# mnastorg/PSI-GNN

Hardware: AMD Instinct MI355X
Metric: fixed-point edges/sec (E' x Broyden iterations/sec) on 1M-node Poisson mesh (higher is better)
Workload: dtype f32

## Files before the change

### psi-gnn_amd/csrc/common.h

```cpp
#pragma once
#include <hip/hip_runtime.h>
#include <stdint.h>
#include <stdio.h>
#include <string>
#include "../../include/psignn_hip.h"

#define D PSIGNN_D

void psignn_set_error(const char* fmt, ...);

extern int g_knob_epoch;
#define KNOB_INT(var, expr)                   \
  static int var##_epoch = -1;                \
  static int var = 0;                         \
  if (var##_epoch != g_knob_epoch) {          \
    var = (expr);                             \
    var##_epoch = g_knob_epoch;               \
  }

#define HIP_TRY(expr)                                                                   \
  do {                                                                                  \
    hipError_t _e = (expr);                                                             \
    if (_e != hipSuccess) {                                                             \
      psignn_set_error("%s:%d: %s -> %s", __FILE__, __LINE__, #expr, hipGetErrorString(_e)); \
// ... 111 lines not shown
    __VA_ARGS__;                         \
    if (g_prof_on) prof_end(st);         \
  } while (0)

#define FLAG_DIRICHLET 1
#define FLAG_NEUMANN 2

struct BatchDesc {
  int64_t M, ld;
  int32_t nblk, npart, nblk_ax, jgroups, thr, seq_len, keep_trace, n_tiles, tile_base;
  int32_t* st;
  float *U, *V, *xbuf, *g0, *g1, *upd, *part, *coef, *nrm_part, *jpart;
  double *rel_trace, *abs_trace;
  const struct TileCtx* ctx;
  const float *h0p, *prbp;
  float* part2;
  int32_t nblk_u, npart_u;
  float* parta;
  int32_t nblk4, pad_;
  const float* nrmp;
  int64_t pstride;
};

static inline size_t tile_lds_min() {
  KNOB_INT(mn, [] { const char* e = getenv("PSIGNN_TILE_LDS_MIN"); return e ? atoi(e) : 0; }());
  return (size_t)(mn < 0 ? 0 : (mn > 65536 ? 65536 : mn));
}
```

### psi-gnn_amd/csrc/fgnn_tile.hip

```cpp
#ifndef MV2_LAUNDER
#define MV2_LAUNDER 2
#endif
#ifndef MV2_CH
#define MV2_CH 10
#endif
#include "tile_helpers.h"
#ifndef TILE_WPE
#define TILE_WPE 0
#endif
#ifndef FUSED_WPE
#define FUSED_WPE 0
#endif
#if FUSED_WPE
#define TILE_WPE_ATTR __attribute__((amdgpu_waves_per_eu(FUSED ? FUSED_WPE : 1, FUSED ? FUSED_WPE : 8)))
#elif TILE_WPE
#define TILE_WPE_ATTR __attribute__((amdgpu_waves_per_eu(TILE_WPE, TILE_WPE)))
#else
#define TILE_WPE_ATTR
#endif
#ifndef X_RELOAD
#define X_RELOAD 1
#endif
#ifndef EDGE_CLAMP
#define EDGE_CLAMP 1
#endif
#ifndef EDGE_BOTH
#define EDGE_BOTH 1
#endif

// ... 38 lines not shown
#include <string.h>
#include <algorithm>
static int stage1_mfma(bool fused, bool mixed) {
  KNOB_INT(forced, [] {
    const char* e = getenv("PSIGNN_STAGE1");
    return !e ? -1 : (strcmp(e, "mfma") == 0 ? 1 : 0);
  }());
  if (forced >= 0) return forced;
  (void)fused;
  (void)mixed;
  return 0;
}

struct FuseArgs {
  const float* upd;
  float* gnew;
  float* xbuf;
  const int32_t* st;
  int off_done, off_cur, off_nxt;
  int64_t M;
  float* part;
  int npart;
  long long* stamps;
};

#ifndef TILE_PRIO
#define TILE_PRIO 15
#endif
#define PRIO_AT(ph) do { if (TILE_PRIO) __builtin_amdgcn_s_setprio((TILE_PRIO >> (2 * (ph))) & 3); } while (0)
#ifndef TILE_STAMPS
#define TILE_STAMPS 0
#endif
#if !TILE_STAMPS
#define STAMP(i) do { } while (0)
#else
#define STAMP(i)                                                                                        \
  do {                                                                                                  \
    if (fa.stamps && (threadIdx.x & 63) == 0)                                                           \
      fa.stamps[((int64_t)tile * 4 + (threadIdx.x >> 6)) * 8 + (i)] = (long long)wall_clock64(); \
  } while (0)
#endif
static long long* g_tile_stamps = nullptr;
extern "C" void psignn_prof_tile_stamps(void* d_buf) { g_tile_stamps = (long long*)d_buf; }

template <int CTRL>
__device__ __forceinline__ float dpp_perm_f(float v) {
// ... 473 lines not shown
  }
}

#ifndef TILE_CTX_VALUE
#define TILE_CTX_VALUE 1
#endif
#if TILE_CTX_VALUE
#define TILE_CTX_PARAM const TileCtx Cv
#define TILE_CTX_USE const TileCtx* __restrict__ C = &Cv;
#else
#define TILE_CTX_PARAM const TileCtx* __restrict__ C
#define TILE_CTX_USE
#endif
template <int P, bool MIXED, bool FUSED, bool MFMA1>
__global__ __launch_bounds__(TILE_THREADS) TILE_WPE_ATTR void k_f_tile(FuseArgs fa, int n_tiles, int chunk, const int32_t* __restrict__ tile_list,
                                                TILE_CTX_PARAM, const float* __restrict__ W, int lofs, int tofs,
                                                int tnofs, int apply_ln, const float* __restrict__ h,
                                                const int32_t* __restrict__ hsel, int64_t hstride,
                                                const float* __restrict__ h0, const float* __restrict__ prb,
                                                const float* __restrict__ nrm, float* __restrict__ out) {
  TILE_CTX_USE
  extern __shared__ __attribute__((aligned(16))) float lds[];
  if (FUSED && fa.st[fa.off_done]) return;
  const int slot = (blockIdx.x & 7) * chunk + (blockIdx.x >> 3);
  if (slot >= n_tiles) return;
  f_tile_body<P, MIXED, FUSED, MFMA1>(fa, slot, tile_list, C, W, lofs, tofs, tnofs, apply_ln, h, hsel, hstride, h0, prb, nrm, out,
                                      lds);
}

static unsigned tile_grid(int chunk);

#ifndef BATCH_WPE
#define BATCH_WPE 0
#endif
#if BATCH_WPE
#define BATCH_WPE_ATTR __attribute__((amdgpu_waves_per_eu(BATCH_WPE, BATCH_WPE)))
#else
#define BATCH_WPE_ATTR
#endif
template <int P, bool MIXED>
__global__ __launch_bounds__(TILE_THREADS) BATCH_WPE_ATTR void k_f_tile_batch(const BatchDesc* __restrict__ descs, int n_mesh, int n_slots, int chunk,
                                                              int off_done, int off_cur, int off_nxt, int par,
                                                              const float* __restrict__ W, int lofs, int tofs, int tnofs) {
  extern __shared__ __attribute__((aligned(16))) float lds[];
  const int slot = (blockIdx.x & 7) * chunk + (blockIdx.x >> 3);
  if (slot >= n_slots) return;
  int m = 0;
  while (m + 1 < n_mesh && descs[m + 1].tile_base <= slot) ++m;
  const BatchDesc& d = descs[m];
  if (d.st[off_done]) return;
  FuseArgs fa{d.upd, par ? d.g0 : d.g1, d.xbuf, d.st, off_done, off_cur, off_nxt, d.M, d.nrm_part, d.n_tiles, nullptr};
  f_tile_body<P, MIXED, true, false>(fa, slot - d.tile_base, nullptr, d.ctx, W, lofs, tofs, tnofs, 1, d.xbuf, nullptr, 0, d.h0p, d.prbp,
                                     d.nrmp, nullptr, lds);
}

int psignn_f_tile_fused_batch(const BatchDesc* d_descs, int n_mesh, int n_slots, int max_rows, const float* W, int mixed,
                              int off_done, int off_cur, int off_nxt, int par, hipStream_t st) {
  const int chunk = (int)cdiv(n_slots, 8);
  if (mixed) {
    using L = WLayout<3>;
    LAUNCH("k_f_tile_fused", st, (k_f_tile_batch<3, true><<<tile_grid(chunk), TILE_THREADS, (size_t)max_rows * TileRow<true>::RS * 4, st>>>(
        d_descs, n_mesh, n_slots, chunk, off_done, off_cur, off_nxt, par, W, L::layer(0), L::tp_layer(1, true, 0), L::tp_neu(1))));
  } else {
    using L = WLayout<2>;
    LAUNCH("k_f_tile_fused", st, (k_f_tile_batch<2, false><<<tile_grid(chunk), TILE_THREADS, (size_t)max_rows * TileRow<false>::RS * 4, st>>>(
        d_descs, n_mesh, n_slots, chunk, off_done, off_cur, off_nxt, par, W, L::layer(0), L::tp_layer(1, false, 0), 0)));
  }
  HIP_TRY(hipGetLastError());
  return PSIGNN_OK;
}

__global__ void k_permute_rows(int64_t N, int cols, const int32_t* __restrict__ map, const float* __restrict__ src,
                               float* __restrict__ dst) {
  int64_t i = (int64_t)blockIdx.x * blockDim.x + threadIdx.x;
// ... 21 lines not shown
      hipMemcpy(tsl.data(), p->tile_slice, (nt + 1) * 4, hipMemcpyDeviceToHost) != hipSuccess ||
      hipMemcpy(hc.data(), p->halo_cnt, nt * 4, hipMemcpyDeviceToHost) != hipSuccess ||
      hipMemcpy(deg.data(), p->slice_deg, p->n_slices, hipMemcpyDeviceToHost) != hipSuccess)
    return nullptr;
  std::vector<int64_t> cost(nt);
  for (int64_t t = 0; t < nt; ++t) {
    int dmax = 0;
    for (int s = tsl[t]; s < tsl[t + 1]; ++s) dmax = std::max(dmax, (int)deg[s]);
    cost[t] = (int64_t)(tptr[t + 1] - tptr[t] + hc[t]) + 16 * (int64_t)dmax;
  }
  for (int64_t t = 0; t < nt; ++t) order[t] = (int32_t)t;
  for (int x = 0; x < 8; ++x) {
    const int64_t a = std::min<int64_t>(nt, (int64_t)x * chunk), b = std::min<int64_t>(nt, (int64_t)(x + 1) * chunk);
    std::stable_sort(order.begin() + a, order.begin() + b, [&](int32_t u, int32_t v) { return cost[u] > cost[v]; });
  }
  int32_t* d = nullptr;
  if (hipMalloc((void**)&d, nt * 4) != hipSuccess) return nullptr;
  if (hipMemcpy(d, order.data(), nt * 4, hipMemcpyHostToDevice) != hipSuccess) { (void)hipFree(d); return nullptr; }
  p->tile_order_cost = d;
  (void)st;
  return d;
}

static FuseArgs plain_args() {
  FuseArgs a{};
  a.stamps = g_tile_stamps;
  return a;
}

template <bool FUSED>
static void launch_mixed(const psignn_plan* p, const FuseArgs& fa, const char* name, const float* W, int nl, const float* h,
                         const int32_t* hsel, int64_t hstride, const float* h0, const float* prb, const float* nrm,
                         float* out, hipStream_t st) {
  using L = WLayout<3>;
  const int lofs = L::layer(nl - 1), tofs = L::tp_layer(nl, true, nl - 1), tnofs = L::tp_neu(nl);
  int na = (int)p->n_tiles_plain, nb = (int)(p->n_tiles - p->n_tiles_plain);
  const char* e = getenv("PSIGNN_MIXED_SPLIT_MIN");
  if (na < (e ? atoi(e) : 2048)) {
    na = 0;
    nb = (int)p->n_tiles;
  }
  const int32_t* list_b = na > 0 ? p->tile_order + na : nullptr;
  if (na > 0) {
    const int chunk = (int)cdiv(na, 8);
    LAUNCH(name, st, (k_f_tile<3, false, FUSED, false><<<tile_grid(chunk), TILE_THREADS, (size_t)p->max_rows * TileRow<false>::RS * 4, st>>>(
        fa, na, chunk, p->tile_order, TILE_ARGS, W, lofs, tofs, tnofs, 1, h, hsel, hstride, h0, prb, nrm, out)));
  }
  if (nb > 0) {
    const int chunk = (int)cdiv(nb, 8);
    LAUNCH(name, st, (k_f_tile<3, true, FUSED, false><<<tile_grid(chunk), TILE_THREADS, (size_t)p->max_rows * TileRow<true>::RS * 4, st>>>(
        fa, nb, chunk, list_b, TILE_ARGS, W, lofs, tofs, tnofs, 1, h, hsel, hstride, h0, prb, nrm, out)));
  }
}

int psignn_f_tile_forward(const psignn_plan* p, const float* W, int nl, const float* h, const int32_t* hsel,
                          int64_t hstride, const float* h0, const float* prb, const float* nrm, float* out,
                          float* work, hipStream_t st) {
  ARG_CHECK(p && p->tiled, "plan has no tile structures");
  ARG_CHECK(W && h && h0 && prb && out, "NULL argument");
  ARG_CHECK(!p->mixed || nrm, "mixed plan needs unit normals");
  const int chunk = (int)cdiv(p->n_tiles, 8);
  const unsigned grid = tile_grid(chunk);
  PROF_BYTES(((p->mixed ? 102 : 89) * p->N + 20 * p->Ep) * (p->mixed ? 1 : nl));
  if (p->mixed) {
    using L = WLayout<3>;
    if (stage1_mfma(false, true)) {
      size_t lds = (size_t)p->max_rows * TileRow<true>::RS * 4;
      LAUNCH("k_f_tile", st, (k_f_tile<3, true, false, true><<<grid, TILE_THREADS, lds, st>>>(
        plain_args(), (int)p->n_tiles, chunk, nullptr, TILE_ARGS, W, L::layer(nl - 1), L::tp_layer(nl, true, nl - 1), L::tp_neu(nl), 1,
        h, hsel, hstride, h0, prb, nrm, out)));
    } else {
      launch_mixed<false>(p, plain_args(), "k_f_tile", W, nl, h, hsel, hstride, h0, prb, nrm, out, st);
    }
// ... 25 lines not shown
                        float* out, hipStream_t st) {
  ARG_CHECK(p && p->tiled && !p->mixed && l >= 0 && l < nl, "tiled layer: dirichlet plans, 0 <= layer < n_layers");
  ARG_CHECK(W && h && h0 && prb && out && out != h, "bad arguments");
  using L = WLayout<2>;
  const int chunk = (int)cdiv(p->n_tiles, 8);
  const unsigned grid = tile_grid(chunk);
  size_t lds = std::max((size_t)p->max_rows * TileRow<false>::RS * 4, tile_lds_min());
  const int32_t* tlist = tile_cost_order(p, chunk, st);
  PROF_BYTES(89 * p->N + 20 * p->Ep);
  if (stage1_mfma(false, false))
    LAUNCH("k_f_tile_layer", st, (k_f_tile<2, false, false, true><<<grid, TILE_THREADS, lds, st>>>(
        plain_args(), (int)p->n_tiles, chunk, tlist, TILE_ARGS, W, L::layer(l), L::tp_layer(nl, false, l), 0, l == nl - 1, h,
        nullptr, 0, h0, prb, nullptr, out)));
  else
    LAUNCH("k_f_tile_layer", st, (k_f_tile<2, false, false, false><<<grid, TILE_THREADS, lds, st>>>(
        plain_args(), (int)p->n_tiles, chunk, tlist, TILE_ARGS, W, L::layer(l), L::tp_layer(nl, false, l), 0, l == nl - 1, h,
        nullptr, 0, h0, prb, nullptr, out)));
  HIP_TRY(hipGetLastError());
  return PSIGNN_OK;
}

int psignn_f_tile_fused(const psignn_plan* p, const float* W, int nl, float* xbuf, int64_t M, const int32_t* st_words,
                        int off_done, int off_cur, int off_nxt, const float* upd, float* gnew,
                        const float* h0, const float* prb, const float* nrm, float* part, hipStream_t st) {
  ARG_CHECK(p && p->tiled, "plan has no tile structures");
  ARG_CHECK(nl == 1 || p->mixed, "fused step supports single-layer evaluation");
  const int chunk = (int)cdiv(p->n_tiles, 8);
  const unsigned grid = tile_grid(chunk);
  const int npart = (int)p->n_tiles;
  FuseArgs fa{upd, gnew, xbuf, st_words, off_done, off_cur, off_nxt, M, part, npart, g_tile_stamps};
  PROF_BYTES((p->mixed ? 102 : 89) * p->N + 20 * p->Ep + 8 * M);
  if (p->mixed) {
    using L = WLayout<3>;
    if (stage1_mfma(true, true)) {
      size_t lds = (size_t)p->max_rows * TileRow<true>::RS * 4;
      LAUNCH("k_f_tile_fused", st, (k_f_tile<3, true, true, true><<<grid, TILE_THREADS, lds, st>>>(
        fa, (int)p->n_tiles, chunk, nullptr, TILE_ARGS, W, L::layer(nl - 1), L::tp_layer(nl, true, nl - 1), L::tp_neu(nl), 1, xbuf,
        nullptr, 0, h0, prb, nrm, nullptr)));
    } else {
      launch_mixed<true>(p, fa, "k_f_tile_fused", W, nl, xbuf, nullptr, 0, h0, prb, nrm, nullptr, st);
    }
  } else {
    using L = WLayout<2>;
    size_t lds = std::max((size_t)p->max_rows * TileRow<false>::RS * 4, tile_lds_min());
    const int32_t* tlist = tile_cost_order(p, chunk, st);
    if (stage1_mfma(true, false))
      LAUNCH("k_f_tile_fused", st, (k_f_tile<2, false, true, true><<<grid, TILE_THREADS, lds, st>>>(
        fa, (int)p->n_tiles, chunk, tlist, TILE_ARGS, W, L::layer(0), L::tp_layer(nl, false, 0), 0, 1, xbuf, nullptr, 0, h0, prb, nrm,
        nullptr)));
    else
      LAUNCH("k_f_tile_fused", st, (k_f_tile<2, false, true, false><<<grid, TILE_THREADS, lds, st>>>(
        fa, (int)p->n_tiles, chunk, tlist, TILE_ARGS, W, L::layer(0), L::tp_layer(nl, false, 0), 0, 1, xbuf, nullptr, 0, h0, prb, nrm,
        nullptr)));
  }
  HIP_TRY(hipGetLastError());
  return npart;
}

extern "C" int psignn_plan_permute(const psignn_plan_t* p, const float* src, int cols, float* dst, int to_plan, void* stream) {
  ARG_CHECK(p && src && dst && cols > 0, "bad arguments");
  ARG_CHECK(src != dst, "in-place permutation is not supported");
  hipStream_t st = (hipStream_t)stream;
  if (!p->tiled) {
    HIP_TRY(hipMemcpyAsync(dst, src, (size_t)p->N * cols * 4, hipMemcpyDeviceToDevice, st));
    return PSIGNN_OK;
  }
  int64_t n = p->N * cols;
// ... 5 lines not shown
```

### psi-gnn_amd/csrc/solver.hip

```cpp
#include "vec_helpers.h"
#include <stdlib.h>
#include <math.h>
#include <algorithm>
#include <vector>

struct Status {
  int32_t n_iter;
  int32_t done;
  int32_t prot_break;
  int32_t stop_reason;
  int32_t lowest_step;
  int32_t cur;
  int32_t low;
  int32_t nxt;
  double lowest_rel, lowest_abs_at;
  double rel0;
  double abs0;
  int32_t lowest_step_abs;
  int32_t stop_abs;
  double s, beta;
};

#define PARTA_LD 32
#ifndef SWEEP_V_AHEAD
#define SWEEP_V_AHEAD 0
#endif
#define RB 256
#define RA 8
struct psignn_broyden {
  const psignn_plan* plan = nullptr;
  int64_t M = 0;
  int seq_len = D;
  int thr = 0;
  int keep_trace = 0;
  int vec = 16;
  int nblk = 0, npart = 0;
  int vec_ax = 0, nblk_ax = 0;
  int jgroups = 1;
  float* jpart = nullptr;
  float *U = nullptr, *V = nullptr;
  float* xbuf = nullptr;
  float* gbuf[2] = {nullptr, nullptr};
  float *upd = nullptr, *fx = nullptr, *fwork = nullptr;
  float* lwork = nullptr;
  int64_t lwork_floats = 0;
  float* nrm_part = nullptr;
  float* part2 = nullptr;
  int uvu = 0;
  int vec_u = 0, nblk_u = 0, npart_u = 0;
  int u2d_kmax = 0, nblk4 = 0, a_ready = 0;
  int u2d_keep = 0, a_from = 0;
// ... 87 lines not shown
__global__ __launch_bounds__(TB) void k_resid(int64_t M, const Status* __restrict__ st, const float* __restrict__ xb,
                                              const float* __restrict__ fx, float* __restrict__ gnew,
                                              float* __restrict__ part, int npart) {
  if (st->done) return;
  int64_t e0 = elem0<VEC>();
  float sg = 0.f, sf = 0.f;
  if (e0 < M) {
    const float* xn = xb + (int64_t)st->nxt * M;
    float x[VEC], f[VEC];
    ldv<VEC>(xn, e0, M, x);
    ldv<VEC>(fx, e0, M, f);
#pragma unroll
    for (int i = 0; i < VEC; ++i) {
      float gn = f[i] - x[i];
      sg = fmaf(gn, gn, sg);
      sf = fmaf(f[i], f[i], sf);
      x[i] = gn;
    }
    stv<VEC>(gnew, e0, M, x);
  }
  block_pair_store(sg, sf, part, npart);
}

__device__ void check_block(Status* st, const float* __restrict__ part, int npart, double* __restrict__ rel_trace,
                            double* __restrict__ abs_trace, double eps, int thr, int seq_len, int keep_trace, double* sh) {
  __shared__ double sh2[RB];
  Status s = *st;
  if (s.done) return;
  double sg, sf;
  block_sum_col2(part, part + npart, npart, sh, sh2, sg, sf);
  if (threadIdx.x != 0) return;
  double abs_diff = (double)(float)sqrt(sg);
  double rel_diff = abs_diff / ((double)(float)sqrt(sf) + 1e-9);
  const int n = s.n_iter + 1;
  s.n_iter = n;
  rel_trace[n - 1] = rel_diff;
  abs_trace[n - 1] = abs_diff;
  if (n == 1) {
    s.rel0 = rel_diff;
    s.abs0 = abs_diff;
  }
  const bool stop_abs = s.stop_abs != 0;
  const bool low_rel = rel_diff < s.lowest_rel, low_abs = abs_diff < s.lowest_abs_at;
  if (low_rel) {
    s.lowest_rel = rel_diff;
    s.lowest_step = n;
// ... 18 lines not shown
  const double obj = stop_abs ? abs_diff : rel_diff;
  const double* tr = stop_abs ? abs_trace : rel_trace;
  int reason = -1;
  if (obj < eps) {
    reason = 1;
  } else if (obj < 3 * eps && n > 30) {
    double mx = obj, mn = obj;
    for (int i = n - 30; i < n - 1; ++i) {
      double r = tr[i];
      mx = r > mx ? r : mx;
      mn = r < mn ? r : mn;
    }
    if (mx / mn < 1.3) reason = 2;
  }
  if (reason < 0 && obj > (stop_abs ? s.abs0 * 1e6 : s.rel0 * 1e3) * seq_len) {
    reason = 3;
    s.prot_break = 1;
  }
  if (reason < 0 && n >= thr) reason = 0;
  if (reason >= 0) {
    s.done = 1;
    s.stop_reason = reason;
  }
  *st = s;
}

#define DOTS_PART4 1
template <int VEC>
__device__ __forceinline__ void dots_body(int64_t M, int k, const Status* __restrict__ st,
                                             const float* __restrict__ U, const float* __restrict__ V,
                                             const float* __restrict__ dxv, const float* __restrict__ dgv,
                                             const float* __restrict__ gv, float* __restrict__ part, int64_t pstride, int ldp,
                                             int jstride, int64_t ld) {
  __shared__ PairStash<3> sh;
  if (__builtin_amdgcn_readfirstlane(st->done)) return;
  const int j0 = blockIdx.y * jstride, j1 = min(k, j0 + jstride);
  if (j0 >= j1) return;
  int64_t e0 = elem0<VEC>();
  float dx[VEC], dg[VEC], g[VEC];
  bool act = e0 < M;
  if (act) {
    ldv<VEC>(dxv, e0, M, dx);
    ldv<VEC>(dgv, e0, M, dg);
    ldv<VEC>(gv, e0, M, g);
#pragma unroll
    for (int i = 0; i < VEC; ++i) dg[i] = g[i] - dg[i];
  } else {
// ... 113 lines not shown
  sweep_u1_body<VEC>(M, k, st, U, dxv, part, ldp, ld);
}
template <int VEC>
__global__ __launch_bounds__(TB) void k_sweep_u1_bf16(int64_t M, int k, const Status* __restrict__ st, const __bf16* __restrict__ U,
                                                      const float* __restrict__ dxv, float* __restrict__ part, int ldp, int64_t ld) {
  sweep_u1_body<VEC, __bf16>(M, k, st, U, dxv, part, ldp, ld);
}

__device__ __forceinline__ void reduce_a_check_body(Status* st, const float* __restrict__ part, int nrows, int ldp, int thr, int k,
                                                    float* __restrict__ coef, const float* __restrict__ nrm_part, int nn,
                                                    double* __restrict__ rel_trace, double* __restrict__ abs_trace,
                                                    double eps, int seq_len, int keep_trace, double* sh,
                                                    const float* __restrict__ parta = nullptr, int nrows4 = 0, int a_from = 1 << 30) {
  if (blockIdx.y == RA) {
    if (blockIdx.x == 0) check_block(st, nrm_part, nn, rel_trace, abs_trace, eps, thr, seq_len, keep_trace, sh);
    return;
  }
  const int done = st->done;
  const int j = blockIdx.x, r = blockIdx.y;
  if (j >= k) return;
  const float* col = j >= a_from ? parta + (j - a_from) : part + j;
  const int n = j >= a_from ? nrows4 : nrows;
  const int64_t stride = j >= a_from ? PARTA_LD : ldp;
  const int lo = (int)((int64_t)n * r / RA), hi = (int)((int64_t)n * (r + 1) / RA);
  const double s = block_sum_col(col + (int64_t)lo * stride, hi - lo, stride, sh);
  if (threadIdx.x == 0 && !done) coef[(3 + r) * thr + j] = (float)s;
}
__global__ __launch_bounds__(RB) void k_reduce_a_check(Status* st, const float* __restrict__ part, int nrows, int ldp, int thr, int k,
                                                       float* __restrict__ coef, const float* __restrict__ nrm_part, int nn,
                                                       double* __restrict__ rel_trace, double* __restrict__ abs_trace,
                                                       double eps, int seq_len, int keep_trace, const float* __restrict__ parta,
                                                       int nrows4, int a_from) {
  __shared__ double sh[RB];
  reduce_a_check_body(st, part, nrows, ldp, thr, k, coef, nrm_part, nn, rel_trace, abs_trace, eps, seq_len, keep_trace, sh, parta, nrows4, a_from);
}

template <int VEC, class P = float>
__device__ __forceinline__ void sweep_v_body(int64_t M, int k, const Status* __restrict__ st, P* __restrict__ V,
                                             const float* __restrict__ dxv, const float* __restrict__ dgv,
                                             const float* __restrict__ gv, const float* __restrict__ coef,
                                             float* __restrict__ part, int64_t pstride, int ldp, float* __restrict__ part2, int nblk, int64_t ld,
                                             int thr) {
  __shared__ PairStash<2> sh;
  if (__builtin_amdgcn_readfirstlane(st->done)) return;
  int64_t e0 = elem0<VEC>();
  float dg[VEC], g[VEC], av[VEC];
  const bool act = e0 < M;
  if (act) {
// ... 99 lines not shown
__device__ __forceinline__ void reduce_cb_body(Status* __restrict__ st, const float* __restrict__ part, int nrows, int64_t pstride, int ldp, int thr, int k,
                                               float* __restrict__ coef, const float* __restrict__ part2, int nblk, double* sh) {
  const int done = st->done;
  if (blockIdx.y == 2) {
    if (blockIdx.x != 0) return;
    __shared__ double sh2[RB];
    double sv, beta;
    block_sum_col2(part2, part2 + nblk, nblk, sh, sh2, sv, beta);
    if (threadIdx.x == 0 && !done) {
      st->s = (double)(float)sv;
      st->beta = (double)(float)beta;
    }
    return;
  }
  const int j = blockIdx.x, c = 1 + blockIdx.y;
  if (j >= k) return;
  const double s = block_sum_col(part + (int64_t)c * pstride + j, nrows, ldp, sh);
  if (threadIdx.x == 0 && !done) coef[c * thr + j] = (float)s;
}
__global__ __launch_bounds__(RB) void k_reduce_cb(Status* __restrict__ st, const float* __restrict__ part, int nrows, int64_t pstride, int ldp, int thr, int k,
                                                  float* __restrict__ coef, const float* __restrict__ part2, int nblk) {
  __shared__ double sh[RB];
  reduce_cb_body(st, part, nrows, pstride, ldp, thr, k, coef, part2, nblk, sh);
}

template <int VEC, class P = float>
__device__ __forceinline__ void sweep_u2_body(int64_t M, int k, const Status* __restrict__ st, P* __restrict__ U,
                                              float* __restrict__ upd, const float* __restrict__ dgv,
                                              const float* __restrict__ gv, const float* __restrict__ coef, int thr, int64_t ld) {
  if (__builtin_amdgcn_readfirstlane(st->done)) return;
  int64_t e0 = elem0<VEC>();
  if (((int64_t)blockIdx.x * TB + (threadIdx.x & ~63)) * VEC >= M) return;
  const bool act = e0 < M;
  float a1[VEC], a2[VEC], dg[VEC];
  if (act) {
    ldv<VEC>(upd, e0, M, a1);
    ldv<VEC>(dgv, e0, M, dg);
    ldv<VEC>(gv, e0, M, a2);
#pragma unroll
    for (int i = 0; i < VEC; ++i) dg[i] = a2[i] - dg[i];
  } else {
#pragma unroll
    for (int i = 0; i < VEC; ++i) a1[i] = a2[i] = dg[i] = 0.f;
  }
#pragma unroll
  for (int i = 0; i < VEC; ++i) a1[i] = a1[i] + dg[i];
// ... 474 lines not shown
                                              float* __restrict__ upd, int64_t ld, const float* __restrict__ part,
                                              int npart) {
  __shared__ double sh[TB];
  final_body<VEC>(M, k, st, U, upd, ld, part, npart, sh);
}

template <int VEC>
__global__ __launch_bounds__(TB) void k_copy_sel(int64_t M, const float* __restrict__ xb, const int32_t* __restrict__ sel,
                                                 int fixed, float* __restrict__ dst) {
  int64_t e0 = elem0<VEC>();
  if (e0 >= M) return;
  int idx = sel ? *sel : fixed;
  float a[VEC];
  ldv<VEC>(xb + (int64_t)idx * M, e0, M, a);
  stv<VEC>(dst, e0, M, a);
}

int psignn_f_eval_p(const psignn_plan_t* p, const float* W, int nl, const float* hbase, const int32_t* d_sel,
                    int64_t stride, const float* h0, const float* prb, const float* nrm, float* out, float* work,
                    hipStream_t st);

int psignn_f_tile_fused(const psignn_plan* p, const float* W, int nl, float* xbuf, int64_t M, const int32_t* st_words,
                        int off_done, int off_cur, int off_nxt, const float* upd, float* gnew,
                        const float* h0, const float* prb, const float* nrm, float* part, hipStream_t st);

#define U2R_KB_MAX 24
#define U2D_LDS_KMAX (PARTA_LD - 1)
static_assert(U2R_KB_MAX + 1 <= PARTA_LD, "the register fold's kept pairs must fit a partials row");
__global__ __launch_bounds__(TB) void kb_sweep_u2d(const BatchDesc* __restrict__ descs, int k, int j_keep0, int par);
static bool u2d_lds_attr(int dev) {
  static int state[64] = {0};
  if (dev < 0 || dev >= 64) return false;
  if (state[dev] == 0) {
    const int want = U2D_LDS_KMAX * TB * 16;
    const bool ok = hipFuncSetAttribute((const void*)k_sweep_u2d, hipFuncAttributeMaxDynamicSharedMemorySize, want) == hipSuccess &&
                    hipFuncSetAttribute((const void*)kb_sweep_u2d, hipFuncAttributeMaxDynamicSharedMemorySize, want) == hipSuccess;
    if (!ok) (void)hipGetLastError();
    state[dev] = ok ? 1 : -1;
  }
  return state[dev] > 0;
}

static int broyden_alloc(psignn_broyden* s) {
  size_t M = (size_t)s->M, thr = (size_t)s->thr;
  const int64_t vec16_min = [] {
    const char* e = getenv("PSIGNN_VEC16_MIN");
    return e ? (int64_t)atoll(e) : (int64_t)3 << 18;
// ... 149 lines not shown
}
extern "C" int psignn_broyden_create_for_batch(psignn_broyden_t** out, const psignn_plan_t* plan, int threshold, int keep_trace,
                                               int64_t shard_elems) {
  ARG_CHECK(out, "out is NULL");
  *out = nullptr;
  ARG_CHECK(plan, "bad arguments");
  return psignn_broyden_create_opts(out, plan, 0, 0, threshold, keep_trace, shard_elems, 0);
}

extern "C" size_t psignn_broyden_bytes(const psignn_broyden_t* s) { return s ? s->bytes : 0; }

extern "C" int psignn_broyden_set_stop_mode(psignn_broyden_t* s, int abs_mode) {
  ARG_CHECK(s, "NULL solver");
  s->stop_abs = abs_mode ? 1 : 0;
  return PSIGNN_OK;
}

static inline int sel_off_cur() { return offsetof(Status, cur) / 4; }
static inline int sel_off_low() { return offsetof(Status, low) / 4; }
static inline int sel_off_nxt() { return offsetof(Status, nxt) / 4; }

static inline __bf16* bf16_pairs(float* p) { return reinterpret_cast<__bf16*>(p); }

static void launch_update(psignn_broyden* s, int k, double eps, hipStream_t st, int fused_npart = 0) {
  unsigned g = (unsigned)s->nblk;
  float* const gnew = s->gbuf[(k + 1) & 1];
  const float* const gold = s->gbuf[k & 1];
  if (!fused_npart) {
    PROF_BYTES(3 * (int64_t)s->M * 4);
    VLAUNCH("k_resid", st, s->vec, k_resid, (g, TB, 0, st), s->M, s->st, s->xbuf, s->fx, gnew, s->nrm_part, s->nblk);
  }
  const int np = fused_npart ? fused_npart : s->nblk;
  if (s->uvu) {
    const int kd = k >= s->thr ? 0 : k;
    const unsigned gu = (unsigned)s->nblk_u;
    if (k == 0) s->a_ready = 0;
    const int a_from = s->a_ready ? s->a_from : kd;
    if (std::min(a_from, kd) > 0 && s->hist) {
      PROF_BYTES((2 * (int64_t)kd + 4) * s->M);
      VLAUNCH("k_sweep_u1_bf16", st, s->vec_u, k_sweep_u1_bf16, (gu, TB, 0, st), s->M, kd, s->st, bf16_pairs(s->U), s->upd, s->part, s->ldp, s->ld);
    } else if (std::min(a_from, kd) > 0) {
      PROF_BYTES((std::min(a_from, kd) + 1) * (int64_t)s->M * 4);
      VLAUNCH("k_sweep_u1", st, s->vec_u, k_sweep_u1, (gu, TB, 0, st), s->M, std::min(a_from, kd), s->st, s->U, s->upd, s->part, s->ldp, s->ld);
    }
    LAUNCH("k_reduce_check", st, (k_reduce_a_check<<<dim3(std::max(kd, 1), RA + 1), RB, 0, st>>>(
        s->st, s->part, s->nblk_u, s->ldp, s->thr, kd, s->coef, s->nrm_part, np, s->rel_trace, s->abs_trace, eps, s->seq_len, s->keep_trace,
        s->parta, s->nblk4, a_from)));
    s->a_ready = 0;
    if (k >= s->thr) return;
    const bool last = k + 1 >= s->thr;
    if (s->hist) {
      PROF_BYTES(last ? 0 : (2 * (int64_t)k + 14) * s->M);
      VLAUNCH("k_sweep_v_bf16", st, s->vec_u, k_sweep_v_bf16, (gu, TB, 0, st), s->M, k, s->st, bf16_pairs(s->V), s->upd, gold, gnew, s->coef, s->part, s->pstride, s->ldp, s->part2, s->nblk_u, s->ld, s->thr);
      LAUNCH("k_reduce_cb", st, (k_reduce_cb<<<dim3(std::max(k, 1), 3), RB, 0, st>>>(s->st, s->part, s->nblk_u, s->pstride, s->ldp, s->thr, k, s->coef, s->part2, s->nblk_u)));
      PROF_BYTES(last ? 0 : (2 * (int64_t)k + 18) * s->M);
      VLAUNCH("k_sweep_u2_bf16", st, s->vec_u, k_sweep_u2_bf16, (gu, TB, 0, st), s->M, k, s->st, bf16_pairs(s->U), s->upd, gold, gnew, s->coef, s->thr, s->ld);
      return;
    }
    PROF_BYTES(last ? 0 : (k + 4) * (int64_t)s->M * 4);
    VLAUNCH("k_sweep_v", st, s->vec_u, k_sweep_v, (gu, TB, 0, st), s->M, k, s->st, s->V, s->upd, gold, gnew, s->coef, s->part, s->pstride, s->ldp, s->part2, s->nblk_u, s->ld, s->thr);
    LAUNCH("k_reduce_cb", st, (k_reduce_cb<<<dim3(std::max(k, 1), 3), RB, 0, st>>>(s->st, s->part, s->nblk_u, s->pstride, s->ldp, s->thr, k, s->coef, s->part2, s->nblk_u)));
    const int keep0 = k <= s->u2d_kmax ? 0 : k - s->u2d_keep;
    if (s->u2d_kmax > 0 && (k <= s->u2d_kmax || s->u2d_keep > 0) && k + 1 < s->thr) {
      PROF_BYTES((k + 5) * (int64_t)s->M * 4);
      const int nk = k - keep0;
      if (s->u2d_reg) {
#define U2R_ARGS s->M, k, s->st, s->U, s->upd, gold, gnew, s->coef, s->thr, s->parta, s->ld, keep0
        if (nk <= 8) LAUNCH("k_sweep_u2d", st, (k_sweep_u2r<8><<<(unsigned)s->nblk4, TB, 0, st>>>(U2R_ARGS)));
        else if (nk <= 16) LAUNCH("k_sweep_u2d", st, (k_sweep_u2r<16><<<(unsigned)s->nblk4, TB, 0, st>>>(U2R_ARGS)));
        else LAUNCH("k_sweep_u2d", st, (k_sweep_u2r<24><<<(unsigned)s->nblk4, TB, 0, st>>>(U2R_ARGS)));
#undef U2R_ARGS
      } else {
        const size_t lds = (size_t)std::max(nk, 1) * TB * 16;
        LAUNCH("k_sweep_u2d", st, (k_sweep_u2d<<<(unsigned)s->nblk4, TB, lds, st>>>(s->M, k, s->st, s->U, s->upd, gold, gnew, s->coef, s->thr, s->parta,
                                                                                    s->ld, keep0)));
      }
      s->a_ready = 1;
      s->a_from = keep0;
    } else {
      PROF_BYTES(last ? 0 : (k + 5) * (int64_t)s->M * 4);
      VLAUNCH("k_sweep_u2", st, s->vec_u, k_sweep_u2, (gu, TB, 0, st), s->M, k, s->st, s->U, s->upd, gold, gnew, s->coef, s->thr, s->ld);
    }
    return;
  }
// ... 69 lines not shown
                                    const float* nrm, double eps, int poll_every, float* d_result,
                                    psignn_solve_info_t* info, double* h_rel, double* h_abs, void* stream) {
  ARG_CHECK(s && s->plan, "solver was not created from a mesh plan");
  ARG_CHECK(W && h0 && prb, "NULL argument");
  ARG_CHECK(!s->plan->mixed || nrm, "mixed plan needs unit normals");
  hipStream_t st = (hipStream_t)stream;
  s->plan_order = 1;
  if (poll_every <= 0) poll_every = 8;
  unsigned g = (unsigned)s->nblk;
  const int32_t* sel_nxt = reinterpret_cast<const int32_t*>(s->st) + sel_off_nxt();
  k_init_status<<<4, TB, 0, st>>>(s->st, s->rel_trace, s->abs_trace, s->thr, s->stop_abs);
  int rc;
  const psignn_plan* p = s->plan;
  if ((rc = psignn_plan_permute(p, h0, D, s->h0p, 1, st))) return rc;
  if ((rc = psignn_plan_permute(p, prb, p->mixed ? 3 : 2, s->prbp, 1, st))) return rc;
  if (p->mixed && (rc = psignn_plan_permute(p, nrm, 2, s->nrmp, 1, st))) return rc;
  const float* nrmp = p->mixed ? s->nrmp : nullptr;
  if ((rc = psignn_f_eval_p(p, W, nl, s->h0p, nullptr, 0, s->h0p, s->prbp, nrmp, s->fx, s->fwork, st))) return rc;
  VPLAIN(s->vec, k_begin, (g, TB, 0, st), s->M, s->h0p, s->fx, s->xbuf, s->gbuf[0], s->upd);
  const bool fused = p->tiled && (nl == 1 || p->mixed);
  const int32_t* st_words = reinterpret_cast<const int32_t*>(s->st);
  KNOB_INT(use_graph, [] { const char* e = getenv("PSIGNN_GRAPH"); return (int)(e && atoi(e) != 0); }());
  if (use_graph && fused && !g_prof_on) {
    uint64_t key = (uint64_t)(uintptr_t)W * 1000003u ^ (uint64_t)(uintptr_t)nrmp * 7919u ^ (uint64_t)nl * 31u ^ (uint64_t)poll_every;
    double e = eps;
    key ^= *reinterpret_cast<uint64_t*>(&e);
    if (key != s->graph_key) {
      for (hipGraphExec_t g : s->graphs)
        if (g) (void)hipGraphExecDestroy(g);
      s->graphs.clear();
      s->graph_key = key;
    }
    const int nchunk = (int)cdiv(s->thr, poll_every);
    s->graphs.resize(nchunk, nullptr);
    for (int c = 0; c < nchunk; ++c) {
      if (!s->graphs[c]) {
        hipGraph_t graph;
        HIP_TRY(hipStreamBeginCapture(st, hipStreamCaptureModeThreadLocal));
        for (int it = c * poll_every; it < std::min(s->thr, (c + 1) * poll_every); ++it) {
          rc = psignn_f_tile_fused(p, W, nl, s->xbuf, s->M, st_words, offsetof(Status, done) / 4, sel_off_cur(), sel_off_nxt(),
                                   s->upd, s->gbuf[(it + 1) & 1], s->h0p, s->prbp, nrmp, s->nrm_part, st);
          if (rc >= 0) launch_update(s, it, eps, st, rc);
        }
        HIP_TRY(hipStreamEndCapture(st, &graph));
        if (rc < 0) return rc;
        HIP_TRY(hipGraphInstantiate(&s->graphs[c], graph, nullptr, nullptr, 0));
        HIP_TRY(hipGraphDestroy(graph));
      }
      HIP_TRY(hipGraphLaunch(s->graphs[c], st));
      rc = read_status(s, st);
      if (rc) return rc;
      if (s->h_st->done) break;
    }
    return finish(s, d_result, info, h_rel, h_abs, st);
  }
  for (int it = 0; it < s->thr; ++it) {
    if (fused) {
      rc = psignn_f_tile_fused(p, W, nl, s->xbuf, s->M, st_words, offsetof(Status, done) / 4, sel_off_cur(),
                               sel_off_nxt(), s->upd, s->gbuf[(it + 1) & 1], s->h0p, s->prbp, nrmp, s->nrm_part, st);
      if (rc < 0) return rc;
      launch_update(s, it, eps, st, rc);
    } else {
      PROF_BYTES(3 * (int64_t)s->M * 4);
      VLAUNCH("k_xnext", st, s->vec, k_xnext, (g, TB, 0, st), s->M, s->st, s->xbuf, s->upd, nullptr);
      rc = psignn_f_eval_p(p, W, nl, s->xbuf, sel_nxt, s->M, s->h0p, s->prbp, nrmp, s->fx, s->fwork, st);
      if (rc) return rc;
      launch_update(s, it, eps, st);
    }
    if ((it + 1) % poll_every == 0 || it + 1 == s->thr) {
      rc = read_status(s, st);
      if (rc) return rc;
      if (s->h_st->done) break;
    }
  }
  return finish(s, d_result, info, h_rel, h_abs, st);
}


static __device__ __forceinline__ int batch_groups(const BatchDesc& d, int k) {
  return (d.jgroups > 1 && k >= 4 * d.jgroups) ? d.jgroups : 1;
}
static __device__ __forceinline__ int idiv_up(int a, int b) { return (a + b - 1) / b; }
static __device__ __forceinline__ const float* bd_gold(const BatchDesc& d, int par) { return par ? d.g1 : d.g0; }
static __device__ __forceinline__ float* bd_gnew(const BatchDesc& d, int par) { return par ? d.g0 : d.g1; }
// ... 517 lines not shown
```

### psi-gnn_amd/csrc/vec_helpers.h

```cpp
#pragma once
#include "common.h"

#define TB 256

#ifndef WAVE_SUM_SHFL
#define WAVE_SUM_SHFL 0
#endif
template <int CTRL>
__device__ __forceinline__ float dpp_perm(float v) {
  return __builtin_bit_cast(float, __builtin_amdgcn_update_dpp(0, __builtin_bit_cast(int, v), CTRL, 0xF, 0xF, true));
}
__device__ __forceinline__ float wave_sum(float v) {
#if WAVE_SUM_SHFL
#pragma unroll
  for (int o = 32; o > 0; o >>= 1) v += __shfl_xor(v, o);
  return v;
#else
  v += dpp_perm<0xB1>(v);
  v += dpp_perm<0x4E>(v);
  v += dpp_perm<0x141>(v);
  v += dpp_perm<0x140>(v);
  const int vi = __builtin_bit_cast(int, v);
  const float r0 = __builtin_bit_cast(float, __builtin_amdgcn_readlane(vi, 0));
  const float r1 = __builtin_bit_cast(float, __builtin_amdgcn_readlane(vi, 16));
// ... 199 lines not shown
    const float y0 = q[i], y1 = q[i + T], y2 = q[i + 2 * T], y3 = q[i + 3 * T];
    a0 += (double)x0; a1 += (double)x1; a2 += (double)x2; a3 += (double)x3;
    b0 += (double)y0; b1 += (double)y1; b2 += (double)y2; b3 += (double)y3;
  }
  for (; i < n; i += T) {
    a0 += (double)p[i];
    b0 += (double)q[i];
  }
  sh[threadIdx.x] = (a0 + a1) + (a2 + a3);
  sh2[threadIdx.x] = (b0 + b1) + (b2 + b3);
  __syncthreads();
  for (int o = T / 2; o > 0; o >>= 1) {
    if ((int)threadIdx.x < o) {
      sh[threadIdx.x] += sh[threadIdx.x + o];
      sh2[threadIdx.x] += sh2[threadIdx.x + o];
    }
    __syncthreads();
  }
  sp = sh[0];
  sq = sh2[0];
  __syncthreads();
}

#define VPLAIN(vec, kern, cfg, ...)                                     \
  do {                                                                  \
    if ((vec) == 16) kern<16><<<VCFG cfg>>>(__VA_ARGS__);               \
    else kern<4><<<VCFG cfg>>>(__VA_ARGS__);                            \
  } while (0)
#define VCFG(...) __VA_ARGS__
#define VLAUNCH(name, st, vec, kern, cfg, ...) LAUNCH(name, st, VPLAIN(vec, kern, cfg, __VA_ARGS__))
```

Baseline: 2.237 billion.

## Fold Broyden a-coefficient reduction into fused tile kernel and merge convergence check

Extra workgroups appended to the fused tile-evaluation grid now compute the a-coefficient column sums from parta, so the separate sweep_u1 and reduce_a_check launches can be skipped when the history is fully in parta. The convergence check block is folded into the later reduce_cb launch, or run as a lone k_check on the final iteration. The aim is fewer kernel launches and dependent serialization points per Broyden iteration. It adds grid tail blocks and LDS floor requirements to the tile kernel, changes when the status is written relative to other reductions, and is gated by an env knob that defaults on.

```diff
diff --git a/psi-gnn_amd/csrc/common.h b/psi-gnn_amd/csrc/common.h
--- a/psi-gnn_amd/csrc/common.h
+++ b/psi-gnn_amd/csrc/common.h
@@ -157,6 +157,12 @@
   int64_t pstride;
 };
 
+struct FuseAJob {
+  const float* parta;
+  float* coef;
+  int nrows4, kd, thr;
+};
+
 static inline size_t tile_lds_min() {
   KNOB_INT(mn, [] { const char* e = getenv("PSIGNN_TILE_LDS_MIN"); return e ? atoi(e) : 0; }());
   return (size_t)(mn < 0 ? 0 : (mn > 65536 ? 65536 : mn));
diff --git a/psi-gnn_amd/csrc/fgnn_tile.hip b/psi-gnn_amd/csrc/fgnn_tile.hip
--- a/psi-gnn_amd/csrc/fgnn_tile.hip
+++ b/psi-gnn_amd/csrc/fgnn_tile.hip
@@ -5,6 +5,8 @@
 #define MV2_CH 10
 #endif
 #include "tile_helpers.h"
+#include "vec_helpers.h"
+static_assert(TILE_THREADS == 256, "the a-reduction workgroups of the fused step sum in k_reduce_a_check's block shape (RB = 256)");
 #ifndef TILE_WPE
 #define TILE_WPE 0
 #endif
@@ -89,6 +91,7 @@
   float* part;
   int npart;
   long long* stamps;
+  FuseAJob aj;
 };
 
 #ifndef TILE_PRIO
@@ -608,6 +611,13 @@
   TILE_CTX_USE
   extern __shared__ __attribute__((aligned(16))) float lds[];
   if (FUSED && fa.st[fa.off_done]) return;
+  const int q = (int)blockIdx.x - 8 * chunk;
+  if (FUSED && q >= 0) {
+    const int j = q / RA, r = q - j * RA;
+    const double s = a_chunk_sum(fa.aj.parta + j, fa.aj.nrows4, PARTA_LD, r, reinterpret_cast<double*>(lds));
+    if (threadIdx.x == 0) fa.aj.coef[(3 + r) * fa.aj.thr + j] = (float)s;
+    return;
+  }
   const int slot = (blockIdx.x & 7) * chunk + (blockIdx.x >> 3);
   if (slot >= n_tiles) return;
   f_tile_body<P, MIXED, FUSED, MFMA1>(fa, slot, tile_list, C, W, lofs, tofs, tnofs, apply_ln, h, hsel, hstride, h0, prb, nrm, out,
@@ -635,7 +645,7 @@
   while (m + 1 < n_mesh && descs[m + 1].tile_base <= slot) ++m;
   const BatchDesc& d = descs[m];
   if (d.st[off_done]) return;
-  FuseArgs fa{d.upd, par ? d.g0 : d.g1, d.xbuf, d.st, off_done, off_cur, off_nxt, d.M, d.nrm_part, d.n_tiles, nullptr};
+  FuseArgs fa{d.upd, par ? d.g0 : d.g1, d.xbuf, d.st, off_done, off_cur, off_nxt, d.M, d.nrm_part, d.n_tiles, nullptr, FuseAJob{}};
   f_tile_body<P, MIXED, true, false>(fa, slot - d.tile_base, nullptr, d.ctx, W, lofs, tofs, tnofs, 1, d.xbuf, nullptr, 0, d.h0p, d.prbp,
                                      d.nrmp, nullptr, lds);
 }
@@ -703,6 +713,8 @@
   return d;
 }
 
+static size_t aj_lds(const FuseArgs& fa, size_t lds) { return fa.aj.kd > 0 ? std::max(lds, (size_t)TILE_THREADS * 8) : lds; }
+
 static FuseArgs plain_args() {
   FuseArgs a{};
   a.stamps = g_tile_stamps;
@@ -722,14 +734,17 @@
     nb = (int)p->n_tiles;
   }
   const int32_t* list_b = na > 0 ? p->tile_order + na : nullptr;
+  const unsigned tail = FUSED ? (unsigned)(fa.aj.kd * RA) : 0u;
   if (na > 0) {
     const int chunk = (int)cdiv(na, 8);
-    LAUNCH(name, st, (k_f_tile<3, false, FUSED, false><<<tile_grid(chunk), TILE_THREADS, (size_t)p->max_rows * TileRow<false>::RS * 4, st>>>(
+    LAUNCH(name, st, (k_f_tile<3, false, FUSED, false><<<tile_grid(chunk) + (nb > 0 ? 0u : tail), TILE_THREADS,
+                                                         aj_lds(fa, (size_t)p->max_rows * TileRow<false>::RS * 4), st>>>(
         fa, na, chunk, p->tile_order, TILE_ARGS, W, lofs, tofs, tnofs, 1, h, hsel, hstride, h0, prb, nrm, out)));
   }
   if (nb > 0) {
     const int chunk = (int)cdiv(nb, 8);
-    LAUNCH(name, st, (k_f_tile<3, true, FUSED, false><<<tile_grid(chunk), TILE_THREADS, (size_t)p->max_rows * TileRow<true>::RS * 4, st>>>(
+    LAUNCH(name, st, (k_f_tile<3, true, FUSED, false><<<tile_grid(chunk) + tail, TILE_THREADS,
+                                                        aj_lds(fa, (size_t)p->max_rows * TileRow<true>::RS * 4), st>>>(
         fa, nb, chunk, list_b, TILE_ARGS, W, lofs, tofs, tnofs, 1, h, hsel, hstride, h0, prb, nrm, out)));
   }
 }
@@ -801,18 +816,20 @@
 
 int psignn_f_tile_fused(const psignn_plan* p, const float* W, int nl, float* xbuf, int64_t M, const int32_t* st_words,
                         int off_done, int off_cur, int off_nxt, const float* upd, float* gnew,
-                        const float* h0, const float* prb, const float* nrm, float* part, hipStream_t st) {
+                        const float* h0, const float* prb, const float* nrm, float* part, hipStream_t st, const FuseAJob* aj) {
   ARG_CHECK(p && p->tiled, "plan has no tile structures");
   ARG_CHECK(nl == 1 || p->mixed, "fused step supports single-layer evaluation");
+  ARG_CHECK(!aj || aj->kd <= 0 || (aj->parta && aj->coef && aj->kd <= PARTA_LD && aj->kd < aj->thr), "bad a-reduction job");
   const int chunk = (int)cdiv(p->n_tiles, 8);
-  const unsigned grid = tile_grid(chunk);
   const int npart = (int)p->n_tiles;
-  FuseArgs fa{upd, gnew, xbuf, st_words, off_done, off_cur, off_nxt, M, part, npart, g_tile_stamps};
+  FuseArgs fa{upd, gnew, xbuf, st_words, off_done, off_cur, off_nxt, M, part, npart, g_tile_stamps, FuseAJob{}};
+  if (aj && aj->kd > 0) fa.aj = *aj;
+  const unsigned grid = tile_grid(chunk) + (unsigned)(fa.aj.kd * RA);
   PROF_BYTES((p->mixed ? 102 : 89) * p->N + 20 * p->Ep + 8 * M);
   if (p->mixed) {
     using L = WLayout<3>;
     if (stage1_mfma(true, true)) {
-      size_t lds = (size_t)p->max_rows * TileRow<true>::RS * 4;
+      size_t lds = aj_lds(fa, (size_t)p->max_rows * TileRow<true>::RS * 4);
       LAUNCH("k_f_tile_fused", st, (k_f_tile<3, true, true, true><<<grid, TILE_THREADS, lds, st>>>(
         fa, (int)p->n_tiles, chunk, nullptr, TILE_ARGS, W, L::layer(nl - 1), L::tp_layer(nl, true, nl - 1), L::tp_neu(nl), 1, xbuf,
         nullptr, 0, h0, prb, nrm, nullptr)));
@@ -821,7 +838,7 @@
     }
   } else {
     using L = WLayout<2>;
-    size_t lds = std::max((size_t)p->max_rows * TileRow<false>::RS * 4, tile_lds_min());
+    size_t lds = aj_lds(fa, std::max((size_t)p->max_rows * TileRow<false>::RS * 4, tile_lds_min()));
     const int32_t* tlist = tile_cost_order(p, chunk, st);
     if (stage1_mfma(true, false))
       LAUNCH("k_f_tile_fused", st, (k_f_tile<2, false, true, true><<<grid, TILE_THREADS, lds, st>>>(
diff --git a/psi-gnn_amd/csrc/solver.hip b/psi-gnn_amd/csrc/solver.hip
--- a/psi-gnn_amd/csrc/solver.hip
+++ b/psi-gnn_amd/csrc/solver.hip
@@ -21,12 +21,10 @@
   double s, beta;
 };
 
-#define PARTA_LD 32
 #ifndef SWEEP_V_AHEAD
 #define SWEEP_V_AHEAD 0
 #endif
 #define RB 256
-#define RA 8
 struct psignn_broyden {
   const psignn_plan* plan = nullptr;
   int64_t M = 0;
@@ -160,6 +158,9 @@
   block_pair_store(sg, sf, part, npart);
 }
 
+struct alignas(8) StatusHead { int64_t w[9]; };
+static_assert(offsetof(Status, s) == sizeof(StatusHead) && offsetof(Status, beta) + sizeof(double) == sizeof(Status),
+              "s, beta must be the last fields of Status");
 __device__ void check_block(Status* st, const float* __restrict__ part, int npart, double* __restrict__ rel_trace,
                             double* __restrict__ abs_trace, double eps, int thr, int seq_len, int keep_trace, double* sh) {
   __shared__ double sh2[RB];
@@ -224,7 +225,7 @@
     s.done = 1;
     s.stop_reason = reason;
   }
-  *st = s;
+  *reinterpret_cast<StatusHead*>(st) = *reinterpret_cast<const StatusHead*>(&s);
 }
 
 #define DOTS_PART4 1
@@ -384,8 +385,7 @@
   const float* col = j >= a_from ? parta + (j - a_from) : part + j;
   const int n = j >= a_from ? nrows4 : nrows;
   const int64_t stride = j >= a_from ? PARTA_LD : ldp;
-  const int lo = (int)((int64_t)n * r / RA), hi = (int)((int64_t)n * (r + 1) / RA);
-  const double s = block_sum_col(col + (int64_t)lo * stride, hi - lo, stride, sh);
+  const double s = a_chunk_sum(col, n, stride, r, sh);
   if (threadIdx.x == 0 && !done) coef[(3 + r) * thr + j] = (float)s;
 }
 __global__ __launch_bounds__(RB) void k_reduce_a_check(Status* st, const float* __restrict__ part, int nrows, int ldp, int thr, int k,
@@ -531,6 +531,24 @@
                                                   float* __restrict__ coef, const float* __restrict__ part2, int nblk) {
   __shared__ double sh[RB];
   reduce_cb_body(st, part, nrows, pstride, ldp, thr, k, coef, part2, nblk, sh);
+}
+
+__global__ __launch_bounds__(RB) void k_reduce_cb_check(Status* st, const float* __restrict__ part, int nrows, int64_t pstride, int ldp, int thr, int k,
+                                                        float* __restrict__ coef, const float* __restrict__ part2, int nblk,
+                                                        const float* __restrict__ nrm_part, int nn, double* __restrict__ rel_trace,
+                                                        double* __restrict__ abs_trace, double eps, int seq_len, int keep_trace) {
+  __shared__ double sh[RB];
+  if (blockIdx.y == 2 && blockIdx.x == 1) {
+    check_block(st, nrm_part, nn, rel_trace, abs_trace, eps, thr, seq_len, keep_trace, sh);
+    return;
+  }
+  reduce_cb_body(st, part, nrows, pstride, ldp, thr, k, coef, part2, nblk, sh);
+}
+
+__global__ __launch_bounds__(RB) void k_check(Status* st, const float* __restrict__ nrm_part, int nn, double* __restrict__ rel_trace,
+                                              double* __restrict__ abs_trace, double eps, int thr, int seq_len, int keep_trace) {
+  __shared__ double sh[RB];
+  check_block(st, nrm_part, nn, rel_trace, abs_trace, eps, thr, seq_len, keep_trace, sh);
 }
 
 template <int VEC, class P = float>
@@ -1051,7 +1069,7 @@
 
 int psignn_f_tile_fused(const psignn_plan* p, const float* W, int nl, float* xbuf, int64_t M, const int32_t* st_words,
                         int off_done, int off_cur, int off_nxt, const float* upd, float* gnew,
-                        const float* h0, const float* prb, const float* nrm, float* part, hipStream_t st);
+                        const float* h0, const float* prb, const float* nrm, float* part, hipStream_t st, const FuseAJob* aj = nullptr);
 
 #define U2R_KB_MAX 24
 #define U2D_LDS_KMAX (PARTA_LD - 1)
@@ -1247,7 +1265,19 @@
 
 static inline __bf16* bf16_pairs(float* p) { return reinterpret_cast<__bf16*>(p); }
 
-static void launch_update(psignn_broyden* s, int k, double eps, hipStream_t st, int fused_npart = 0) {
+enum { FOLD_OFF = 0, FOLD_FAST = 1, FOLD_MOOT = 2 };
+static int fold_knob() {
+  KNOB_INT(on, [] { const char* e = getenv("PSIGNN_FOLD_REDUCE"); return (int)(!e || atoi(e) != 0); }());
+  return on;
+}
+static int fold_mode(const psignn_broyden* s, int k) {
+  if (!fold_knob() || !s->uvu || s->hist) return FOLD_OFF;
+  if (k + 1 >= s->thr) return FOLD_MOOT;
+  const int a_from = (k > 0 && s->a_ready) ? s->a_from : k;
+  return std::min(a_from, k) == 0 ? FOLD_FAST : FOLD_OFF;
+}
+
+static void launch_update(psignn_broyden* s, int k, double eps, hipStream_t st, int fused_npart = 0, int fold = FOLD_OFF) {
   unsigned g = (unsigned)s->nblk;
   float* const gnew = s->gbuf[(k + 1) & 1];
   const float* const gold = s->gbuf[k & 1];
@@ -1261,16 +1291,23 @@
     const unsigned gu = (unsigned)s->nblk_u;
     if (k == 0) s->a_ready = 0;
     const int a_from = s->a_ready ? s->a_from : kd;
-    if (std::min(a_from, kd) > 0 && s->hist) {
-      PROF_BYTES((2 * (int64_t)kd + 4) * s->M);
-      VLAUNCH("k_sweep_u1_bf16", st, s->vec_u, k_sweep_u1_bf16, (gu, TB, 0, st), s->M, kd, s->st, bf16_pairs(s->U), s->upd, s->part, s->ldp, s->ld);
-    } else if (std::min(a_from, kd) > 0) {
-      PROF_BYTES((std::min(a_from, kd) + 1) * (int64_t)s->M * 4);
-      VLAUNCH("k_sweep_u1", st, s->vec_u, k_sweep_u1, (gu, TB, 0, st), s->M, std::min(a_from, kd), s->st, s->U, s->upd, s->part, s->ldp, s->ld);
-    }
-    LAUNCH("k_reduce_check", st, (k_reduce_a_check<<<dim3(std::max(kd, 1), RA + 1), RB, 0, st>>>(
-        s->st, s->part, s->nblk_u, s->ldp, s->thr, kd, s->coef, s->nrm_part, np, s->rel_trace, s->abs_trace, eps, s->seq_len, s->keep_trace,
-        s->parta, s->nblk4, a_from)));
+    if (fold == FOLD_MOOT) {
+      LAUNCH("k_reduce_check", st, (k_check<<<1, RB, 0, st>>>(s->st, s->nrm_part, np, s->rel_trace, s->abs_trace, eps, s->thr, s->seq_len, s->keep_trace)));
+      s->a_ready = 0;
+      return;
+    }
+    if (fold == FOLD_OFF) {
+      if (std::min(a_from, kd) > 0 && s->hist) {
+        PROF_BYTES((2 * (int64_t)kd + 4) * s->M);
+        VLAUNCH("k_sweep_u1_bf16", st, s->vec_u, k_sweep_u1_bf16, (gu, TB, 0, st), s->M, kd, s->st, bf16_pairs(s->U), s->upd, s->part, s->ldp, s->ld);
+      } else if (std::min(a_from, kd) > 0) {
+        PROF_BYTES((std::min(a_from, kd) + 1) * (int64_t)s->M * 4);
+        VLAUNCH("k_sweep_u1", st, s->vec_u, k_sweep_u1, (gu, TB, 0, st), s->M, std::min(a_from, kd), s->st, s->U, s->upd, s->part, s->ldp, s->ld);
+      }
+      LAUNCH("k_reduce_check", st, (k_reduce_a_check<<<dim3(std::max(kd, 1), RA + 1), RB, 0, st>>>(
+          s->st, s->part, s->nblk_u, s->ldp, s->thr, kd, s->coef, s->nrm_part, np, s->rel_trace, s->abs_trace, eps, s->seq_len, s->keep_trace,
+          s->parta, s->nblk4, a_from)));
+    }
     s->a_ready = 0;
     if (k >= s->thr) return;
     const bool last = k + 1 >= s->thr;
@@ -1284,7 +1321,11 @@
     }
     PROF_BYTES(last ? 0 : (k + 4) * (int64_t)s->M * 4);
     VLAUNCH("k_sweep_v", st, s->vec_u, k_sweep_v, (gu, TB, 0, st), s->M, k, s->st, s->V, s->upd, gold, gnew, s->coef, s->part, s->pstride, s->ldp, s->part2, s->nblk_u, s->ld, s->thr);
-    LAUNCH("k_reduce_cb", st, (k_reduce_cb<<<dim3(std::max(k, 1), 3), RB, 0, st>>>(s->st, s->part, s->nblk_u, s->pstride, s->ldp, s->thr, k, s->coef, s->part2, s->nblk_u)));
+    if (fold == FOLD_FAST)
+      LAUNCH("k_reduce_check", st, (k_reduce_cb_check<<<dim3(std::max(k, 2), 3), RB, 0, st>>>(s->st, s->part, s->nblk_u, s->pstride, s->ldp, s->thr, k,
+          s->coef, s->part2, s->nblk_u, s->nrm_part, np, s->rel_trace, s->abs_trace, eps, s->seq_len, s->keep_trace)));
+    else
+      LAUNCH("k_reduce_cb", st, (k_reduce_cb<<<dim3(std::max(k, 1), 3), RB, 0, st>>>(s->st, s->part, s->nblk_u, s->pstride, s->ldp, s->thr, k, s->coef, s->part2, s->nblk_u)));
     const int keep0 = k <= s->u2d_kmax ? 0 : k - s->u2d_keep;
     if (s->u2d_kmax > 0 && (k <= s->u2d_kmax || s->u2d_keep > 0) && k + 1 < s->thr) {
       PROF_BYTES((k + 5) * (int64_t)s->M * 4);
@@ -1400,7 +1441,8 @@
   const int32_t* st_words = reinterpret_cast<const int32_t*>(s->st);
   KNOB_INT(use_graph, [] { const char* e = getenv("PSIGNN_GRAPH"); return (int)(e && atoi(e) != 0); }());
   if (use_graph && fused && !g_prof_on) {
-    uint64_t key = (uint64_t)(uintptr_t)W * 1000003u ^ (uint64_t)(uintptr_t)nrmp * 7919u ^ (uint64_t)nl * 31u ^ (uint64_t)poll_every;
+    uint64_t key = (uint64_t)(uintptr_t)W * 1000003u ^ (uint64_t)(uintptr_t)nrmp * 7919u ^ (uint64_t)nl * 31u ^ (uint64_t)poll_every ^
+                   (uint64_t)fold_knob() << 40;
     double e = eps;
     key ^= *reinterpret_cast<uint64_t*>(&e);
     if (key != s->graph_key) {
@@ -1416,9 +1458,11 @@
         hipGraph_t graph;
         HIP_TRY(hipStreamBeginCapture(st, hipStreamCaptureModeThreadLocal));
         for (int it = c * poll_every; it < std::min(s->thr, (c + 1) * poll_every); ++it) {
+          const int fold = fold_mode(s, it);
+          const FuseAJob aj{s->parta, s->coef, s->nblk4, fold == FOLD_FAST ? it : 0, s->thr};
           rc = psignn_f_tile_fused(p, W, nl, s->xbuf, s->M, st_words, offsetof(Status, done) / 4, sel_off_cur(), sel_off_nxt(),
-                                   s->upd, s->gbuf[(it + 1) & 1], s->h0p, s->prbp, nrmp, s->nrm_part, st);
-          if (rc >= 0) launch_update(s, it, eps, st, rc);
+                                   s->upd, s->gbuf[(it + 1) & 1], s->h0p, s->prbp, nrmp, s->nrm_part, st, &aj);
+          if (rc >= 0) launch_update(s, it, eps, st, rc, fold);
         }
         HIP_TRY(hipStreamEndCapture(st, &graph));
         if (rc < 0) return rc;
@@ -1434,10 +1478,12 @@
   }
   for (int it = 0; it < s->thr; ++it) {
     if (fused) {
+      const int fold = fold_mode(s, it);
+      const FuseAJob aj{s->parta, s->coef, s->nblk4, fold == FOLD_FAST ? it : 0, s->thr};
       rc = psignn_f_tile_fused(p, W, nl, s->xbuf, s->M, st_words, offsetof(Status, done) / 4, sel_off_cur(),
-                               sel_off_nxt(), s->upd, s->gbuf[(it + 1) & 1], s->h0p, s->prbp, nrmp, s->nrm_part, st);
+                               sel_off_nxt(), s->upd, s->gbuf[(it + 1) & 1], s->h0p, s->prbp, nrmp, s->nrm_part, st, &aj);
       if (rc < 0) return rc;
-      launch_update(s, it, eps, st, rc);
+      launch_update(s, it, eps, st, rc, fold);
     } else {
       PROF_BYTES(3 * (int64_t)s->M * 4);
       VLAUNCH("k_xnext", st, s->vec, k_xnext, (g, TB, 0, st), s->M, s->st, s->xbuf, s->upd, nullptr);
diff --git a/psi-gnn_amd/csrc/vec_helpers.h b/psi-gnn_amd/csrc/vec_helpers.h
--- a/psi-gnn_amd/csrc/vec_helpers.h
+++ b/psi-gnn_amd/csrc/vec_helpers.h
@@ -245,6 +245,13 @@
   __syncthreads();
 }
 
+#define RA 8
+#define PARTA_LD 32
+__device__ inline double a_chunk_sum(const float* __restrict__ col, int n, int64_t stride, int r, double* sh) {
+  const int lo = (int)((int64_t)n * r / RA), hi = (int)((int64_t)n * (r + 1) / RA);
+  return block_sum_col(col + (int64_t)lo * stride, hi - lo, stride, sh);
+}
+
 #define VPLAIN(vec, kern, cfg, ...)                                     \
   do {                                                                  \
     if ((vec) == 16) kern<16><<<VCFG cfg>>>(__VA_ARGS__);               \
```

Result: no change. 2.244 billion, median of 6 (+0.3%).
